# yassouali/pytorch-segmentation

Measured on NVIDIA H100. Metric: images/sec DeepLabV3+/ResNet101 513x513 train step (fwd+CE+bwd+SGD), higher is better.
Workload: dtype bf16

## Files before the change

### include/seg_b200.h

```cpp
#ifndef SEG_B200_H
#define SEG_B200_H

#include <stdint.h>

#ifdef __cplusplus
extern "C" {
#endif

#define SEG_DT_BF16 0
#define SEG_DT_F32 1

#define SEG_IMPL_AUTO 0
#define SEG_IMPL_SIMT 1
#define SEG_IMPL_TC 2

typedef struct seg_conv_desc {
  int32_t N, H, W, C;
  int32_t K;
  int32_t R, S;
  int32_t stride, pad, dil;
  int32_t P, Q;
  int32_t ldx;
  int32_t ldy;
} seg_conv_desc;

typedef struct seg_sync_desc {
  void* const* peers;
  int32_t rank, world, n_max;
  int64_t timeout_clocks;
} seg_sync_desc;

const char* seg_last_error(void);
int seg_version(void);
int seg_device_ok(void);
int64_t seg_launch_count(void);
void seg_launch_count_reset(void);

int seg_conv2d_fwd(const seg_conv_desc* d, const void* x, const void* w_packed, void* y, int y_dtype,
                   const float* bias, float beta, double* stats, const seg_sync_desc* sync, void* sync_ticket,
                   int impl, void* stream);
int seg_conv2d_dgrad(const seg_conv_desc* d, const void* dy, const void* w_packed, void* dx, float beta,
                     int impl, void* stream);
int64_t seg_conv2d_wgrad_workspace_floats(const seg_conv_desc* d, int impl);
int seg_conv2d_wgrad(const seg_conv_desc* d, const void* dy, const void* x, float* dw_packed, float* workspace, int impl,
                     void* stream);

int64_t seg_dwconv_scratch_floats(int C);
int seg_dwconv3x3_fwd(const seg_conv_desc* d, const void* x, const float* w9, void* y, double* stats,
                      const seg_sync_desc* sync, void* sync_ticket, void* stream);
int seg_dwconv3x3_bwd_data(const seg_conv_desc* d, const void* dy, const float* w9, void* dx, float beta, void* stream);
int seg_dwconv3x3_bwd_weight(const seg_conv_desc* d, const void* dy, const void* x, float* dw9, float beta,
                             float* scratch, void* stream);
int seg_dw_pack_weight(const float* w_c133, float* w9, int C, void* stream);
int seg_dw_unpack_wgrad(const float* g9, float* g_c133, int C, float beta, void* stream);

int seg_pack_weight(const float* w_oihw, void* w_packed, int K, int C, int R, int S, int Cpad, void* stream);
int seg_unpack_wgrad(const float* dw_packed, float* g_oihw, int K, int C, int R, int S, int Cpad, float beta,
                     void* stream);
int seg_pack_entry_bytes(void);
int seg_pack_weights_batched(const void* table, int n, int64_t total, void* stream);
int seg_unpack_wgrads_batched(const void* table, int n, int64_t total, float beta, void* stream);
int seg_im2col(const seg_conv_desc* d, const void* x, int x_nchw_f32, void* col, int Kpad, void* stream);

int seg_bn_stats(const void* x, int64_t M, int C, int ldx, double* stats, const seg_sync_desc* sync, void* sync_ticket,
                 void* stream);
int seg_bn_finalize(const double* stats, double count, int C, const float* gamma, const float* beta, float eps,
                    float momentum, int clamp_eps, float* running_mean, float* running_var, float* scale_shift,
                    float* save_mean_istd, void* stream);
// ... 177 lines not shown
```

### pytorch-segmentation_b200/csrc/seg_api.cu

```cuda
#include <stdarg.h>
#include "seg_common.cuh"
#include "seg_sync.cuh"

namespace seg {

static thread_local char g_err[1024] = "";
std::atomic<long long> g_launches{0};

void set_error(const char* fmt, ...) {
  va_list ap;
  va_start(ap, fmt);
  vsnprintf(g_err, sizeof(g_err), fmt, ap);
  va_end(ap);
}

namespace tc {
bool supported(const seg_conv_desc* d);
int conv_fwd(const seg_conv_desc* d, const void* x, const void* w, void* y, int y_dtype, const float* bias, float beta,
             double* stats, unsigned* stat_ticket, const seg_sync_desc* sync, cudaStream_t stream);
int conv_dgrad(const seg_conv_desc* d, const void* dy, const void* w, void* dx, float beta, cudaStream_t stream);
int conv_wgrad(const seg_conv_desc* d, const void* dy, const void* x, float* dw, float* ws, cudaStream_t stream);
int64_t wgrad_workspace_floats(const seg_conv_desc* d);
}
namespace simt {
int conv_fwd(const seg_conv_desc* d, const void* x, const void* w, void* y, int y_dtype, const float* bias, float beta,
             double* stats, unsigned* stat_ticket, const seg_sync_desc* sync, cudaStream_t stream);
int conv_dgrad(const seg_conv_desc* d, const void* dy, const void* w, void* dx, float beta, cudaStream_t stream);
int conv_wgrad(const seg_conv_desc* d, const void* dy, const void* x, float* dw, cudaStream_t stream);
}

static int check_desc(const seg_conv_desc* d) {
  SEG_REQUIRE(d != nullptr, "null conv descriptor");
  SEG_REQUIRE(d->N > 0 && d->H > 0 && d->W > 0 && d->C > 0 && d->K > 0 && d->R > 0 && d->S > 0, "bad conv dims");
  SEG_REQUIRE(d->stride >= 1 && d->dil >= 1 && d->pad >= 0, "bad conv stride/dil/pad");
  const int P = (d->H + 2 * d->pad - d->dil * (d->R - 1) - 1) / d->stride + 1;
  const int Q = (d->W + 2 * d->pad - d->dil * (d->S - 1) - 1) / d->stride + 1;
  SEG_REQUIRE(P == d->P && Q == d->Q, "conv output size mismatch: expected %dx%d got %dx%d", P, Q, d->P, d->Q);
  SEG_REQUIRE(d->ldx >= d->C && d->ldy >= d->K, "conv pitch smaller than channel count");
  return 0;
}

static bool tma_base_ok(const void* p) { return (reinterpret_cast<uintptr_t>(p) & 15) == 0; }

}

// ... 43 lines not shown
  const bool tc_ok = tc::supported(d) && d->ldy % 8 == 0 && tma_base_ok(dy) && tma_base_ok(w_packed);
  if (impl == SEG_IMPL_TC || (impl == SEG_IMPL_AUTO && tc_ok))
    return tc::conv_dgrad(d, dy, w_packed, dx, beta, ST(stream));
  return simt::conv_dgrad(d, dy, w_packed, dx, beta, ST(stream));
}

static bool wgrad_on_tc(const seg_conv_desc* d, int impl) {
  return impl == SEG_IMPL_TC || (impl == SEG_IMPL_AUTO && tc::supported(d) && d->ldy % 8 == 0);
}

int64_t seg_conv2d_wgrad_workspace_floats(const seg_conv_desc* d, int impl) {
  if (check_desc(d)) return -1;
  return wgrad_on_tc(d, impl) ? tc::wgrad_workspace_floats(d) : 0;
}

int seg_conv2d_wgrad(const seg_conv_desc* d, const void* dy, const void* x, float* dw_packed, float* workspace, int impl,
                     void* stream) {
  if (check_desc(d)) return 1;
  if (wgrad_on_tc(d, impl) && (impl == SEG_IMPL_TC || (tma_base_ok(dy) && tma_base_ok(x))))
    return tc::conv_wgrad(d, dy, x, dw_packed, workspace, ST(stream));
  return simt::conv_wgrad(d, dy, x, dw_packed, ST(stream));
}

}
```

### pytorch-segmentation_b200/csrc/seg_conv_tc.cu

```cuda
#include <cuda.h>
#include <mutex>
#include <stdlib.h>
#include "seg_common.cuh"
#include "seg_ptx.cuh"
#include "seg_sync.cuh"

namespace seg {
namespace tc {

using namespace ptx;

constexpr int BM = 128;
constexpr int BK = 64;
constexpr int A_BYTES = BM * 128;
constexpr int KIND_KK = 0, KIND_KM = 1;
constexpr int NTHREADS = 384;
constexpr int NCONS = 256;
constexpr int MAXT = 49;

constexpr int BAR_CONSUMERS = 1;
constexpr int BAR_ORDER = 2;
constexpr int BAR_WG = 4;

struct TcParams {
// ... 352 lines not shown
        }
        atomicAdd(p.stats + n0 + tid, (double)a);
        atomicAdd(p.stats + p.Ncols + n0 + tid, (double)b);
      }
    }
  }

  if (p.stats && p.sync.world > 0)
    sync_push_when_last<false>(p.sync, p.stats, 2 * p.Ncols, p.stat_ticket, gridDim.x, threadIdx.x - 128, NCONS,
                               [] { named_sync(BAR_CONSUMERS, NCONS); }, flag_sm);
}


template <int BN>
struct Cfg {
  static constexpr int B_BYTES = BN * 128;
  static constexpr int STAGE_BYTES = A_BYTES + B_BYTES;
  static constexpr int STAGES = BN == 64 ? 6 : (BN == 128 ? 5 : 4);
  static constexpr int SMEM = STAGES * STAGE_BYTES + 1024  + 256 ;
  static_assert(STAGES * STAGE_BYTES >= BM * BN * 4, "staging tile must fit in the pipeline ring");
  static_assert(SMEM <= 227 * 1024, "shared memory per block");
};

template <int BN>
__global__ void __launch_bounds__(NTHREADS, 1) conv_gemm_wgrad(const __grid_constant__ TcParams p) {
  using C = Cfg<BN>;
  constexpr int STAGES = C::STAGES;
  extern __shared__ uint8_t smem_raw[];
  const uint32_t raw_addr = smem_u32(smem_raw);
  const uint32_t smem0 = (raw_addr + 1023u) & ~1023u;
  uint8_t* smem_gen = smem_raw + (smem0 - raw_addr);
  const uint32_t bar0 = smem0 + STAGES * C::STAGE_BYTES;
  auto full_bar = [&](int s) { return bar0 + 8u * s; };
  auto empty_bar = [&](int s) { return bar0 + 8u * (STAGES + s); };

  const int m0 = blockIdx.x * BM;
  const int n0 = blockIdx.y * BN;

  const int tap_mm = blockIdx.z % p.taps;
  const int split = blockIdx.z / p.taps;
  const int kb_begin = split * p.kblocks_per_split;
  const int kb_end = min(kb_begin + p.kblocks_per_split, p.kblocks_total);
  const int num_iters = max(kb_end - kb_begin, 0);

  if (threadIdx.x == 0) {
    prefetch_tmap(&p.mapA);
    prefetch_tmap(&p.mapB);
    for (int s = 0; s < STAGES; ++s) {
      mbar_init(full_bar(s), 1);
      mbar_init(empty_bar(s), 8);
    }
    fence_mbar_init();
  }
  __syncthreads();
  pdl_wait();

  if (threadIdx.x < 128) {
    if (threadIdx.x == 0 && num_iters > 0) {
      const uint16_t oh = (uint16_t)p.tap_oh[tap_mm], ow = (uint16_t)p.tap_ow[tap_mm];
      int it = 0;
      for (int kb = kb_begin; kb < kb_end; ++kb, ++it) {
        const int st = it % STAGES;
        const uint32_t ph = (it / STAGES) & 1;
// ... 156 lines not shown
    SEG_REQUIRE(e == cudaSuccess, "cudaFuncSetAttribute(smem=%d): %s", PPCfg<BN>::SMEM, cudaGetErrorString(e));
    attr_set = true;
  }
  const int n_tiles = ceil_div(p.Ncols, BN);
  const int64_t tiles = ceil_div64(p.M, BM) * n_tiles;
  SEG_REQUIRE(tiles < (1ll << 31), "too many output tiles");
  p.n_tiles = n_tiles;
  p.tiles = (int)tiles;
  const dim3 grid((unsigned)std::min<int64_t>(tiles, num_sms()));
  launch_pdl(kfn, grid, dim3(NTHREADS), (size_t)PPCfg<BN>::SMEM, stream, p);
  return check_launch("conv_gemm_pp");
}

template <int KIND>
static int launch_pp_bn(int bn, TcParams& p, cudaStream_t stream) {
  switch (bn) {
    case 64: return launch_pp<64, KIND>(p, stream);
    case 128: return launch_pp<128, KIND>(p, stream);
  }
  set_error("bad BN %d", bn);
  return 1;
}

template <int BN>
static int launch_wgrad(const TcParams& p, dim3 grid, cudaStream_t stream) {
  static bool attr_set = false;
  auto kfn = conv_gemm_wgrad<BN>;
  if (!attr_set) {
    cudaError_t e = cudaFuncSetAttribute(kfn, cudaFuncAttributeMaxDynamicSharedMemorySize, Cfg<BN>::SMEM);
    SEG_REQUIRE(e == cudaSuccess, "cudaFuncSetAttribute(smem=%d): %s", Cfg<BN>::SMEM, cudaGetErrorString(e));
    attr_set = true;
  }
  launch_pdl(kfn, grid, dim3(NTHREADS), (size_t)Cfg<BN>::SMEM, stream, p);
  return check_launch("conv_gemm_wgrad");
}

static int launch_wgrad_bn(int bn, const TcParams& p, dim3 grid, cudaStream_t stream) {
  switch (bn) {
    case 64: return launch_wgrad<64>(p, grid, stream);
    case 128: return launch_wgrad<128>(p, grid, stream);
    case 256: return launch_wgrad<256>(p, grid, stream);
  }
  set_error("bad BN %d", bn);
  return 1;
}

static int pick_bn(int ncols, bool out_f32) { return (ncols <= 64 || out_f32) ? 64 : 128; }

static int stat_rows_for(int ncols) {
  if (ncols <= 64) return 32;
  if (ncols < 256) return 64;
  return ceil_div(ncols, 256) * 256 - ncols < 128 ? 128 : 64;
}

bool supported(const seg_conv_desc* d) {
  if (d->C % 8 != 0 || d->ldx % 8 != 0) return false;
  if (d->R != d->S) return false;
  if (d->R * d->S > MAXT) return false;
  if (d->pad > 127 || d->dil * (d->R - 1) - d->pad > 127 || d->dil * (d->R - 1) - d->pad < -127) return false;
  if (d->stride > 8) return false;
  return true;
}

static bool is_pointwise(const seg_conv_desc* d) { return d->R == 1 && d->S == 1 && d->stride == 1 && d->pad == 0; }
// ... 131 lines not shown
    dw[i] += acc;
  }
}

static void wgrad_plan(const seg_conv_desc* d, int& bn, int& splits, int& kblocks_per_split) {
  const bool wide = d->R * d->S >= 9 && d->C >= 256 && d->C % 256 == 0;
  bn = (d->C <= 64) ? 64 : (wide ? 256 : 128);
  const int kblocks_total = (int)ceil_div64((int64_t)d->N * d->P * d->Q, BK);
  const int tiles = ceil_div(d->K, BM) * ceil_div(d->C, bn) * d->R * d->S;
  splits = max(1, num_sms() / tiles);
  splits = min(splits, kblocks_total);
  splits = min(splits, 1024);
  kblocks_per_split = ceil_div(kblocks_total, splits);
  splits = ceil_div(kblocks_total, kblocks_per_split);
}

int64_t wgrad_workspace_floats(const seg_conv_desc* d) {
  if (!supported(d)) return 0;
  int bn, splits, kps;
  wgrad_plan(d, bn, splits, kps);
  return splits > 1 ? (int64_t)splits * d->R * d->S * d->K * d->C : 0;
}

int conv_wgrad(const seg_conv_desc* d, const void* dy, const void* x, float* dw, float* ws, cudaStream_t stream) {
  SEG_REQUIRE(supported(d) && d->ldy % 8 == 0, "wgmma conv wgrad: unsupported shape");
  TcParams p;
  memset(&p, 0, sizeof(p));
  const int64_t npix = (int64_t)d->N * d->P * d->Q;
  SEG_REQUIRE(npix < (1ll << 31), "too many pixels");
  p.M = d->K;
  p.Ncols = d->C;
  p.taps = d->R * d->S;
  for (int t = 0; t < p.taps; ++t) {
    p.tap_wt[t] = (short)t;
    p.tap_oh[t] = (short)((t / d->S) * d->dil);
    p.tap_ow[t] = (short)((t % d->S) * d->dil);
  }
  p.stride = d->stride;
  p.lower_h = p.lower_w = -d->pad;
  p.PQ = d->P * d->Q;
  p.Q = d->Q;
  p.dw = dw;
  p.dw_K = d->K;
  p.dw_C = d->C;
  p.kblocks_total = (int)ceil_div64(npix, BK);
  int bn, splits;
  wgrad_plan(d, bn, splits, p.kblocks_per_split);
  SEG_REQUIRE(splits == 1 || ws != nullptr, "wgmma conv wgrad: %d k-splits need the workspace (seg_conv2d_wgrad_workspace_floats)", splits);
  SEG_REQUIRE((int64_t)(splits - 1) * p.kblocks_per_split < p.kblocks_total, "wgmma conv wgrad: split %d has no k-blocks", splits - 1);
  if (splits > 1) p.ws = ws;
  if (make_map_2d(&p.mapA, dy, npix, d->K, d->ldy, 64)) return 1;
  if (is_pointwise(d)) {
    p.x_im2col = 0;
    if (make_map_2d(&p.mapB, x, npix, d->C, d->ldx, 64)) return 1;
  } else {
    p.x_im2col = 1;
    const int upper = d->pad - (d->R - 1) * d->dil;
    if (make_map_im2col(&p.mapB, x, d->N, d->H, d->W, d->C, d->ldx, -d->pad, -d->pad, upper, upper, d->stride, 64)) return 1;
  }
  SEG_REQUIRE((unsigned)(p.taps * splits) <= 65535u, "wgrad grid.z too large");
  dim3 grid((unsigned)ceil_div(d->K, BM), (unsigned)ceil_div(d->C, bn), (unsigned)(p.taps * splits));
  if (launch_wgrad_bn(bn, p, grid, stream)) return 1;
  if (splits == 1) return 0;
  const int64_t n = (int64_t)p.taps * d->K * d->C;
  wgrad_split_reduce_kernel<<<(unsigned)std::min<int64_t>(ceil_div64(n, 256), (int64_t)num_sms() * 8), 256, 0, stream>>>(ws, splits, n, dw);
  return check_launch("wgrad_split_reduce");
}

}
}
```

### pytorch-segmentation_b200/seg_b200/engine.py

```python
import torch

from . import ops
from .lib import IMPL_AUTO, IMPL_TC

BN_EPS = 1e-5
BN_MOM = 0.1
FUSED_BWD_MAX_BYTES = 24 << 20
ACT_DTYPE = torch.bfloat16


class Act:
    __slots__ = ("t", "grad", "needs_grad", "_written")

    def __init__(self, t, needs_grad=True):
        self.t = t
        self.grad = None
        self.needs_grad = needs_grad
        self._written = False

    @property
    def shape(self):
        return self.t.shape

    def grad_target(self):
# ... 54 lines not shown
        return self._packed


class DwSpec:

    def __init__(self, name, module):
        self.name, self.m = name, module
        assert module.groups == module.in_channels == module.out_channels and module.kernel_size == (3, 3)
        self.C = module.in_channels
        self._packed, self._version = None, None
        self.always_repack = False

    stride = property(lambda self: self.m.stride[0])
    pad = property(lambda self: self.m.padding[0])
    dil = property(lambda self: self.m.dilation[0])

    def packed(self):
        w = self.m.weight
        key = (w._version, w.data_ptr())
        if self._packed is None or self._version != key or self.always_repack:
            self._packed = ops.dw_pack_weight(w.detach())
            self._version = key
        return self._packed


class Tape:
    def __init__(self, training, record=None, grads=None, impl=IMPL_AUTO, dropout=True, seed=0, sync=None, clamp_eps=False,
                 step_ctr=None, arena_floats=0, owner=None):
        self.training = training
        self.record = training if record is None else record
        self.back = []
        self.back_params = {}
        self.grads = grads if grads is not None else {}
        self.touched = set()
        self.impl = impl
        self.dropout = dropout
        self.seed = seed
        self.sync = sync
        self.step_ctr = step_ctr
        self.packed_override = {}
        self.dw_buffers = {}
        self.clamp_eps = clamp_eps
        self._drop_ctr = 0
        self._pushed = set()
        self.bn_modules = []
        self.owner = owner
# ... 28 lines not shown
            return
        self.touched.add(p)
        if p in self.grads:
            value_fn(self.grads[p], 1.0)
        else:
            g = torch.empty(p.shape, dtype=torch.float32, device=p.device)
            value_fn(g, 0.0)
            self.grads[p] = g

    def _push_back(self, fn, params=()):
        if params:
            self.back_params[len(self.back)] = tuple(p for p in params if p is not None)
        self.back.append(fn)

    def backward(self, after=None):
        for i in range(len(self.back) - 1, -1, -1):
            self.back[i]()
            if after is not None:
                after(i)
        if self.owner is not None and self.arena_used:
            self.owner._arena_floats = self.arena_used
        self.back = []

    def conv(self, x, spec, out=None, out_dtype=None, want_stats=False, use_bias=True):
        wp = self.packed_override.get(spec)
        if wp is None:
            wp = spec.packed()
        bias = spec.m.bias if use_bias else None
        stats = None
        if out_dtype is None:
            out_dtype = ACT_DTYPE
        want = want_stats and self.training
        sync = tk = None
        if want:
            stats = self.zalloc64(2 * spec.K, wp.device)
            if self.sync_fused():
                sync, tk = self.sync, self.zalloc(1, wp.device)
        if spec.explicit:
            nchw = not isinstance(x, Act)
            if not nchw and self.record and x.needs_grad and (spec.R, spec.S, spec.stride, spec.pad) != (1, 1, 1, 0):
                raise NotImplementedError(f"{spec.name}: data gradient of an im2col conv is built for 1x1 convs only")
            src = x if nchw else x.t
            col = ops.im2col(src, spec.R, spec.S, spec.stride, spec.pad, spec.dil, spec.kpad, nchw_f32=nchw)
            y = ops.conv2d_fwd(col, wp, spec.K, 1, 1, out=out, out_dtype=out_dtype, bias=bias.detach() if bias is not None else None,
                               stats=stats, impl=self.impl, sync=sync, sync_ticket=tk)
            xin, geo = col, (1, 1, 1, 0, 1)
        else:
            y = ops.conv2d_fwd(x.t, wp, spec.K, spec.R, spec.S, spec.stride, spec.pad, spec.dil, out=out, out_dtype=out_dtype,
                               bias=bias.detach() if bias is not None else None, stats=stats, impl=self.impl, sync=sync, sync_ticket=tk)
            xin, geo = x.t, (spec.R, spec.S, spec.stride, spec.pad, spec.dil)
        ya = Act(y)
        if sync is not None:
            self._pushed.add(stats.data_ptr())
        if self.record:
            def bwd():
                dy = ya.grad
                if dy is None:
                    return
                R, S, stride, pad, dil = geo
                if spec.m.weight.requires_grad and spec in self.dw_buffers:
                    ops.conv2d_wgrad(dy, xin, R, S, stride, pad, dil, out=self.dw_buffers[spec], impl=self.impl)
                    self.touched.add(spec.m.weight)
                elif spec.m.weight.requires_grad:
                    dwp = ops.conv2d_wgrad(dy, xin, R, S, stride, pad, dil, impl=self.impl)
                    if spec.explicit:
                        def fill(g, beta):
                            full = dwp[0, :, : spec.R * spec.S * spec.C].reshape(spec.K, spec.R, spec.S, spec.C).permute(0, 3, 1, 2)
                            if beta:
                                g.add_(full)
                            else:
                                g.copy_(full)
                    else:
                        def fill(g, beta):
                            ops.unpack_wgrad(dwp, tuple(spec.m.weight.shape), beta=beta, out=g)
                    self._param_grad(spec.m.weight, fill)
                if bias is not None and bias.requires_grad:
                    cpad = ops.ld(dy)
                    wide = dy if dy.shape[-1] % 8 == 0 else dy.as_strided(dy.shape[:-1] + (cpad,), dy.stride(), dy.storage_offset())
                    s = ops.bn_stats(wide)[: spec.K].float()
                    self._param_grad(bias, lambda g, beta: g.add_(s) if beta else g.copy_(s))
                if (not spec.explicit) and isinstance(x, Act) and x.needs_grad:
                    gx, beta = x.grad_target()
                    ops.conv2d_dgrad(dy, wp, tuple(x.t.shape), R, S, stride, pad, dil, out=gx, beta=beta, impl=self.impl)
                elif isinstance(x, Act) and x.needs_grad:
                    assert x.grad is None, "the input of an im2col conv must have a single consumer"
                    x.grad = ops.conv2d_dgrad(dy, wp, tuple(xin.shape), 1, 1, 1, 0, 1, impl=self.impl)[..., : spec.C]
                    x._written = True
                ya.grad = None
            self._push_back(bwd, (spec.m.weight, bias))
        return ya, stats

    def conv_transpose(self, x, spec, out=None):
        assert spec.transposed
        wp = self.packed_override.get(spec)
        if wp is None:
            wp = spec.packed()
        impl = IMPL_TC if self.impl == IMPL_AUTO else self.impl
        k, s, p = spec.R, spec.stride, spec.pad
        N, h, w, _ = x.t.shape
        y_shape = (N, (h - 1) * s - 2 * p + k, (w - 1) * s - 2 * p + k, spec.C)
        y = ops.conv2d_dgrad(x.t, wp, y_shape, k, k, s, p, 1, out=out, impl=impl)
        ya = Act(y)
        if self.record:
            def bwd():
                dy = ya.grad
                if dy is None:
                    return
                if spec.m.weight.requires_grad and spec in self.dw_buffers:
                    ops.conv2d_wgrad(x.t, dy, k, k, s, p, 1, out=self.dw_buffers[spec], impl=impl)
                    self.touched.add(spec.m.weight)
                elif spec.m.weight.requires_grad:
                    dwp = ops.conv2d_wgrad(x.t, dy, k, k, s, p, 1, impl=impl)
# ... 422 lines not shown
```

### pytorch-segmentation_b200/seg_b200/lib.py

```python
import ctypes
import os
from ctypes import POINTER, Structure, c_char_p, c_double, c_float, c_int, c_int32, c_int64, c_uint8, c_uint32, c_uint64, c_void_p

import torch

_HERE = os.path.dirname(os.path.abspath(__file__))
LIB_PATH = os.path.join(os.path.dirname(_HERE), "libseg_b200.so")

DT_BF16, DT_F32 = 0, 1
IMPL_AUTO, IMPL_SIMT, IMPL_TC = 0, 1, 2
LOSS_CE, LOSS_WCE, LOSS_FOCAL = 0, 1, 2


class SyncDesc(Structure):

    _fields_ = [("peers", c_void_p), ("rank", c_int32), ("world", c_int32), ("n_max", c_int32), ("timeout_clocks", c_int64)]


class ConvDesc(Structure):

    _fields_ = [(n, c_int32) for n in ("N", "H", "W", "C", "K", "R", "S", "stride", "pad", "dil", "P", "Q", "ldx", "ldy")]


def conv_out_size(size, k, stride, pad, dil):
    return (size + 2 * pad - dil * (k - 1) - 1) // stride + 1


def make_conv_desc(N, H, W, C, K, R, S, stride, pad, dil, ldx=None, ldy=None):
    P = conv_out_size(H, R, stride, pad, dil)
    Q = conv_out_size(W, S, stride, pad, dil)
    return ConvDesc(N, H, W, C, K, R, S, stride, pad, dil, P, Q, ldx if ldx is not None else C, ldy if ldy is not None else K)


_SIGS = {
    "seg_last_error": (c_char_p, []),
    "seg_version": (c_int, []),
    "seg_device_ok": (c_int, []),
    "seg_launch_count": (c_int64, []),
    "seg_launch_count_reset": (None, []),
    "seg_conv2d_fwd": (c_int, [POINTER(ConvDesc), c_void_p, c_void_p, c_void_p, c_int, c_void_p, c_float, c_void_p, c_void_p, c_void_p, c_int, c_void_p]),
    "seg_conv2d_dgrad": (c_int, [POINTER(ConvDesc), c_void_p, c_void_p, c_void_p, c_float, c_int, c_void_p]),
    "seg_conv2d_wgrad_workspace_floats": (c_int64, [POINTER(ConvDesc), c_int]),
    "seg_conv2d_wgrad": (c_int, [POINTER(ConvDesc), c_void_p, c_void_p, c_void_p, c_void_p, c_int, c_void_p]),
    "seg_dwconv_scratch_floats": (c_int64, [c_int]),
    "seg_dwconv3x3_fwd": (c_int, [POINTER(ConvDesc), c_void_p, c_void_p, c_void_p, c_void_p, c_void_p, c_void_p, c_void_p]),
    "seg_dwconv3x3_bwd_data": (c_int, [POINTER(ConvDesc), c_void_p, c_void_p, c_void_p, c_float, c_void_p]),
    "seg_dwconv3x3_bwd_weight": (c_int, [POINTER(ConvDesc), c_void_p, c_void_p, c_void_p, c_float, c_void_p, c_void_p]),
    "seg_dw_pack_weight": (c_int, [c_void_p, c_void_p, c_int, c_void_p]),
    "seg_dw_unpack_wgrad": (c_int, [c_void_p, c_void_p, c_int, c_float, c_void_p]),
    "seg_pack_weight": (c_int, [c_void_p, c_void_p, c_int, c_int, c_int, c_int, c_int, c_void_p]),
    "seg_unpack_wgrad": (c_int, [c_void_p, c_void_p, c_int, c_int, c_int, c_int, c_int, c_float, c_void_p]),
    "seg_pack_entry_bytes": (c_int, []),
    "seg_pack_weights_batched": (c_int, [c_void_p, c_int, c_int64, c_void_p]),
    "seg_unpack_wgrads_batched": (c_int, [c_void_p, c_int, c_int64, c_float, c_void_p]),
    "seg_im2col": (c_int, [POINTER(ConvDesc), c_void_p, c_int, c_void_p, c_int, c_void_p]),
    "seg_bn_stats": (c_int, [c_void_p, c_int64, c_int, c_int, c_void_p, c_void_p, c_void_p, c_void_p]),
    "seg_bn_finalize": (c_int, [c_void_p, c_double, c_int, c_void_p, c_void_p, c_float, c_float, c_int, c_void_p, c_void_p, c_void_p, c_void_p, c_void_p]),
    "seg_bn_eval_scale_shift": (c_int, [c_int, c_void_p, c_void_p, c_void_p, c_void_p, c_float, c_void_p, c_void_p, c_void_p]),
    "seg_bn_apply": (c_int, [c_void_p, c_int, c_void_p, c_void_p, c_int, c_void_p, c_int, c_int64, c_int, c_int, c_float, c_uint64, c_void_p, c_int, c_void_p]),
    "seg_counter_add": (c_int, [c_void_p, c_uint64, c_void_p]),
    "seg_bn_bwd_reduce_slots": (c_int, []),
    "seg_bn_bwd_reduce": (c_int, [c_void_p, c_int, c_void_p, c_int, c_void_p, c_void_p, c_int, c_void_p, c_int64, c_int, c_int, c_float, c_void_p, c_void_p, c_void_p, c_void_p, c_void_p, c_int, c_void_p, c_void_p, c_void_p, c_void_p]),
    "seg_bn_apply_train": (c_int, [c_void_p, c_int, c_void_p, c_double, c_void_p, c_void_p, c_float, c_float, c_int, c_void_p, c_void_p, c_void_p, c_void_p, c_int, c_void_p, c_int, c_void_p, c_int64, c_int, c_int, c_float, c_uint64, c_void_p, c_int, c_void_p]),
    "seg_bn_bwd_fused_workspace": (c_int, [c_int64, c_int, POINTER(c_int64), POINTER(c_int64)]),
    "seg_bn_bwd_fused": (c_int, [c_void_p, c_int, c_void_p, c_int, c_void_p, c_void_p, c_int, c_void_p, c_void_p, c_void_p, c_double, c_int64, c_int, c_int, c_float,
                                 c_void_p, c_void_p, c_void_p, c_void_p, c_void_p, c_int, c_void_p, c_int, c_void_p, c_int, c_float, c_int, c_void_p, c_void_p]),
# ... 137 lines not shown
```

### pytorch-segmentation_b200/seg_b200/nets.py

```python
import logging
import math
import weakref
from itertools import chain

import numpy as np
import torch
import torch.nn as nn

from . import ops
from .engine import Act, BilinearHead, ConvSpec, DwSpec, FullResHead, ShuffleHead, Tape
from .lib import IMPL_AUTO, require_device

try:
    from base import BaseModel as _RefBaseModel
except Exception:
    _RefBaseModel = None


_LIVE_MODELS = weakref.WeakSet()


def release_all_graphs():
    import gc
    for m in list(_LIVE_MODELS):
        if hasattr(m, "release_graphs"):
            m.release_graphs()
    gc.collect()
    if torch.cuda.is_available():
        torch.cuda.synchronize()


class BaseModel(nn.Module if _RefBaseModel is None else _RefBaseModel):
    def __init__(self):
# ... 409 lines not shown
                               res=skip if last else None)
        return h

    def _new_tape(self, training, record):
        ctr = None
        if training:
            dev = next(self.parameters()).device
            if self._step_ctr is None or self._step_ctr.device != dev:
                bns = self._flat()[2]
                start = bns[0].num_batches_tracked.detach().reshape(1).to(dev, torch.int64) if bns else None
                self._step_ctr = start.clone() if start is not None else torch.zeros(1, dtype=torch.int64, device=dev)
            ctr = self._step_ctr
            ops.counter_add(ctr, 1)
        return Tape(training, record=record, impl=self.conv_impl, dropout=self.engine_dropout, seed=self._seed(),
                    sync=self.bn_sync, clamp_eps=self.syncbn_clamp_eps, step_ctr=ctr,
                    arena_floats=getattr(self, "_arena_floats", 0) if training else 0, owner=self)

    def _seed(self):
        if self.engine_seed is None:
            rank = torch.distributed.get_rank() if (torch.distributed.is_available() and torch.distributed.is_initialized()) else 0
            self.engine_seed = (int(torch.initial_seed()) * 2654435761 + rank * 0x9E3779B1) & 0x7FFFFFFF
        return self.engine_seed

    def _cbr(self, tape, x, name, conv, bn, relu=True, res=None, out=None, drop_p=0.0, drop_channelwise=False):
        y, st = tape.conv(x, self._spec(name, conv), want_stats=True)
        return tape.bn_act(y, bn, st, relu=relu, res=res, out=out, drop_p=drop_p, drop_channelwise=drop_channelwise)

    def _block(self, tape, x, prefix, blk, out=None):
        a = self._cbr(tape, x, prefix + "conv1", blk.conv1, blk.bn1)
        a = self._cbr(tape, a, prefix + "conv2", blk.conv2, blk.bn2)
        r = x
        if blk.downsample is not None:
            r = self._cbr(tape, x, prefix + "downsample.0", blk.downsample[0], blk.downsample[1], relu=False)
        return self._cbr(tape, a, prefix + "conv3", blk.conv3, blk.bn3, relu=True, res=r, out=out)

    def _finish(self, tape):
        if tape.bn_modules:
            torch._foreach_add_([m.num_batches_tracked for m in tape.bn_modules], 1)

    def _dp_world(self):
        if not self.dp_reduce:
            return 1
        from .comm import dp_world
        return dp_world()

    def _attach_sync_bn(self):
        from . import comm
        if self.use_sync_bn and self.bn_sync is None and comm.dp_world() > 1:
# ... 106 lines not shown
            a = self._xblock(tape, a, f"backbone.block{i}.", getattr(bb, f"block{i}"), relu_out=True)
        for n in (3, 4, 5):
            a = self._sep_unit(tape, a, f"backbone.conv{n}", getattr(bb, f"conv{n}"), getattr(bb, f"bn{n}"), relu_after=True)
        return a, low

    def _trunk_resnet(self, tape, x):
        bb = self.backbone
        a = self._cbr(tape, x, "backbone.layer0.0", bb.layer0[0], bb.layer0[1])
        a = tape.maxpool(a)
        low = None
        for li in (1, 2, 3, 4):
            layer = getattr(bb, f"layer{li}")
            for bi, blk in enumerate(layer):
                a = self._block(tape, a, f"backbone.layer{li}.{bi}.", blk)
            if li == 1:
                low = a
        return a, low

    def _aspp(self, tape, a):
        N, Hf, Wf = a.t.shape[0], a.t.shape[1], a.t.shape[2]
        A = self.ASSP
        cat, sl = tape.concat(N, Hf, Wf, [256] * 5, a.t.device)
        br = []
        for i in (1, 2, 3, 4):
            seq = getattr(A, f"aspp{i}")
            br.append(self._cbr(tape, a, f"ASSP.aspp{i}.0", seq[0], seq[1], out=sl[i - 1]))
        g = tape.avgpool(a, 1)
        g = self._cbr(tape, g, "ASSP.avg_pool.1", A.avg_pool[1], A.avg_pool[2])
        br.append(tape.bilinear(g, Hf, Wf, True, out=sl[4]))
        tape.bind_slices(cat, br)
        return self._cbr(tape, cat, "ASSP.conv1", A.conv1, A.bn1, drop_p=A.dropout.p)

    def _decoder(self, tape, f, low):
        D = self.decoder
        N, Hl, Wl = low.t.shape[0], low.t.shape[1], low.t.shape[2]
        cat2, sl2 = tape.concat(N, Hl, Wl, [48, 256], low.t.device)
        l48 = self._cbr(tape, low, "decoder.conv1", D.conv1, D.bn1, out=sl2[0])
        up = tape.bilinear(f, Hl, Wl, True, out=sl2[1])
        tape.bind_slices(cat2, [l48, up])
        y = self._cbr(tape, cat2, "decoder.output.0", D.output[0], D.output[1])
        y = self._cbr(tape, y, "decoder.output.3", D.output[3], D.output[4], drop_p=D.output[6].p)
        lo, _ = tape.conv(y, self._spec("decoder.output.7", D.output[7]), out_dtype=torch.float32)
        return lo

    def _features(self, tape, x):
        a, low = self._trunk_xception(tape, x) if self.backbone_name == "xception" else self._trunk_resnet(tape, x)
        return self._decoder(tape, self._aspp(tape, a), low)

    def _forward_heads(self, tape, x):
# ... 242 lines not shown
            for p in self.backbone.parameters():
                p.requires_grad = False

    def _decoder(self, tape, f, low):
        D = self.decoder
        N, Hl, Wl = low.t.shape[0], low.t.shape[1], low.t.shape[2]
        cat, sl = tape.concat(N, Hl, Wl, [48, 256], low.t.device)
        l48 = self._cbr(tape, low, "decoder.conv1", D.conv1, D.bn1, out=sl[0])
        u = self._cbr(tape, f, "decoder.DUC.conv", D.DUC.conv, D.DUC.bn)
        up = tape.pixel_shuffle(u, 2, out=sl[1], crop=(Hl, Wl))
        tape.bind_slices(cat, [l48, up])
        y = self._cbr(tape, cat, "decoder.output.0", D.output[0], D.output[1])
        y = self._cbr(tape, y, "decoder.output.3", D.output[3], D.output[4], drop_p=D.output[6].p)
        C = self.num_classes
        buf = torch.empty((N, Hl, Wl, (C + 7) // 8 * 8), dtype=y.t.dtype, device=y.t.device)[..., :C]
        lo, _ = tape.conv(y, self._spec("decoder.output.7", D.output[7]), out=buf)
        return lo

    def _aspp(self, tape, a):
        N, Hf, Wf = a.t.shape[0], a.t.shape[1], a.t.shape[2]
        A = self.ASSP
        cat, sl = tape.concat(N, Hf, Wf, [256] * 7, a.t.device)
        br = []
        for i in range(1, 7):
            seq = getattr(A, f"aspp{i}")
            br.append(self._cbr(tape, a, f"ASSP.aspp{i}.0", seq[0], seq[1], out=sl[i - 1]))
        g = tape.avgpool(a, 1)
        g = self._cbr(tape, g, "ASSP.avg_pool.1", A.avg_pool[1], A.avg_pool[2])
        br.append(tape.bilinear(g, Hf, Wf, True, out=sl[6]))
        tape.bind_slices(cat, br)
        return self._cbr(tape, cat, "ASSP.conv1", A.conv1, A.bn1, drop_p=A.dropout.p)

    def _forward_heads(self, tape, x):
        bb = self.backbone
        a = self._cbr(tape, x, "backbone.layer0.0", bb.layer0[0], bb.layer0[1])
        a = tape.maxpool(a)
        low = None
        for li in (1, 2, 3, 4):
            for bi, blk in enumerate(getattr(bb, f"layer{li}")):
                a = self._block(tape, a, f"backbone.layer{li}.{bi}.", blk)
            if li == 1:
                low = a
        y = self._decoder(tape, self._aspp(tape, a), low)
        z = self._cbr(tape, y, "DUC_out.conv", self.DUC_out.conv, self.DUC_out.bn)
        return [ShuffleHead(z, 4)]

    def get_backbone_params(self):
        return self.backbone.parameters()

# ... 297 lines not shown
```

### pytorch-segmentation_b200/seg_b200/ops.py

```python
import ctypes

import torch

from . import lib
from .lib import DT_BF16, DT_F32, IMPL_AUTO, IMPL_SIMT, IMPL_TC, ConvDesc, call, make_conv_desc, ptr

_IMPL_OVERRIDE = None
PROFILE = None


def _meta(d):
    if lib.TRACE is None:
        return None
    return (d.N, d.H, d.W, d.C, d.K, d.R, d.stride, d.dil, 2.0 * d.N * d.P * d.Q * d.K * d.C * d.R * d.S)


def _meta_rows(M, C, passes, flag=0):
    if lib.TRACE is None:
        return None
    return (int(M), int(C), int(flag), 0, 0, 0, 0, 0, 2.0 * M * C * passes)


def _prof(kind, d):
    if PROFILE is None:
        return None
    e0, e1 = torch.cuda.Event(enable_timing=True), torch.cuda.Event(enable_timing=True)
    flops = 2.0 * d.N * d.P * d.Q * d.K * d.C * d.R * d.S
    nbytes = 2.0 * (d.N * d.H * d.W * d.C + d.N * d.P * d.Q * d.K) + (4.0 if kind == "wgrad" else 2.0) * d.K * d.C * d.R * d.S
    PROFILE.append((kind, flops, e0, e1, nbytes))
    e0.record()
    return e1


def set_conv_impl(impl):
    global _IMPL_OVERRIDE
    _IMPL_OVERRIDE = impl


def _impl(impl):
    return _IMPL_OVERRIDE if _IMPL_OVERRIDE is not None else impl


def ld(t):
    assert t.stride(-1) == 1, "channel dim must be contiguous"
    if t.dim() == 4:
        n, h, w, c = t.shape
        pitch = t.stride(2) if w > 1 else (t.stride(1) // w if h > 1 else (t.stride(0) // (h * w) if n > 1 else c))
        assert w == 1 or t.stride(2) == pitch
        assert h == 1 or t.stride(1) == w * pitch, "rows must be dense"
        assert n == 1 or t.stride(0) == h * w * pitch, "images must be dense"
        return pitch
# ... 73 lines not shown
    ev = _prof("dgrad", d)
    call("seg_conv2d_dgrad", ctypes.byref(d), ptr(dy), ptr(w_packed), ptr(out), float(beta), _impl(impl), meta=_meta(d))
    if ev is not None:
        ev.record()
    return out


def conv2d_wgrad(dy, x, R, S, stride=1, pad=0, dil=1, out=None, impl=IMPL_AUTO):
    N, H, W, C = x.shape
    K = dy.shape[-1]
    if out is None:
        out = torch.zeros((R * S, K, C), dtype=torch.float32, device=x.device)
    d = make_conv_desc(N, H, W, C, K, R, S, stride, pad, dil, ldx=ld(x), ldy=ld(dy))
    assert (d.P, d.Q) == (dy.shape[1], dy.shape[2])
    nws = lib.load().seg_conv2d_wgrad_workspace_floats(ctypes.byref(d), _impl(impl))
    if nws < 0:
        raise RuntimeError(f"seg_conv2d_wgrad_workspace_floats failed: {lib.last_error()}")
    ws = torch.empty(nws, dtype=torch.float32, device=x.device) if nws > 0 else None
    ev = _prof("wgrad", d)
    call("seg_conv2d_wgrad", ctypes.byref(d), ptr(dy), ptr(x), ptr(out), ptr(ws), _impl(impl), meta=_meta(d))
    if ev is not None:
        ev.record()
    return out


def dw_pack_weight(w_c133):
    C = w_c133.shape[0]
    w9 = torch.empty((9, C), dtype=torch.float32, device=w_c133.device)
    call("seg_dw_pack_weight", ptr(w_c133), ptr(w9), C)
    return w9


def dw_unpack_wgrad(g9, out, beta=0.0):
    call("seg_dw_unpack_wgrad", ptr(g9), ptr(out), g9.shape[1], float(beta))
    return out


def _dw_desc(x_shape, stride, pad, dil, ldx, ldy):
    N, H, W, C = x_shape
    return make_conv_desc(N, H, W, C, C, 3, 3, stride, pad, dil, ldx=ldx, ldy=ldy)


def dwconv_fwd(x, w9, stride=1, pad=1, dil=1, out=None, stats=None, sync=None, sync_ticket=None):
    N, H, W, C = x.shape
    d = _dw_desc(x.shape, stride, pad, dil, ld(x), C)
    if out is None:
# ... 652 lines not shown
```

Measured before the change: 383.1.

## Batch ASPP dilated-branch weight gradients into one grouped wgrad launch

Adds a grouped weight-gradient GEMM kernel that packs up to six same-shape conv problems, each with its own dy, pad, dilation and output, into one grid, with blockIdx.z mapped to the member problem. The ASPP 3x3 dilated branches share the same input, so their wgrads are deferred until the last branch's backward runs and are then issued as a single launch. The goal is to fill the GPU better on small per-branch wgrad grids and to cut launch overhead. The cost is a larger grid-constant parameter block, a linear search over groups in each block, and more complex backward bookkeeping for deferral and parameter ownership.

Result: no change. 385.5, median of 6 (+0.6%).

```diff
diff --git a/include/seg_b200.h b/include/seg_b200.h
--- a/include/seg_b200.h
+++ b/include/seg_b200.h
@@ -44,6 +44,10 @@
 int64_t seg_conv2d_wgrad_workspace_floats(const seg_conv_desc* d, int impl);
 int seg_conv2d_wgrad(const seg_conv_desc* d, const void* dy, const void* x, float* dw_packed, float* workspace, int impl,
                      void* stream);
+#define SEG_WGRAD_GROUP_MAX 6
+int64_t seg_conv2d_wgrad_group_workspace_floats(const seg_conv_desc* d, int G, int impl);
+int seg_conv2d_wgrad_group(const seg_conv_desc* d, int G, const void* const* dy, const void* x, float* const* dw_packed,
+                           float* workspace, int impl, void* stream);
 
 int64_t seg_dwconv_scratch_floats(int C);
 int seg_dwconv3x3_fwd(const seg_conv_desc* d, const void* x, const float* w9, void* y, double* stats,
diff --git a/pytorch-segmentation_b200/csrc/seg_api.cu b/pytorch-segmentation_b200/csrc/seg_api.cu
--- a/pytorch-segmentation_b200/csrc/seg_api.cu
+++ b/pytorch-segmentation_b200/csrc/seg_api.cu
@@ -21,6 +21,10 @@
 int conv_dgrad(const seg_conv_desc* d, const void* dy, const void* w, void* dx, float beta, cudaStream_t stream);
 int conv_wgrad(const seg_conv_desc* d, const void* dy, const void* x, float* dw, float* ws, cudaStream_t stream);
 int64_t wgrad_workspace_floats(const seg_conv_desc* d);
+bool wgrad_group_compatible(const seg_conv_desc* d, int G);
+int64_t wgrad_group_workspace_floats(const seg_conv_desc* d, int G);
+int conv_wgrad_group(const seg_conv_desc* d, int G, const void* const* dy, const void* x, float* const* dw, float* ws,
+                     cudaStream_t stream);
 }
 namespace simt {
 int conv_fwd(const seg_conv_desc* d, const void* x, const void* w, void* y, int y_dtype, const float* bias, float beta,
@@ -110,4 +114,39 @@
   return simt::conv_wgrad(d, dy, x, dw_packed, ST(stream));
 }
 
+static bool wgrad_group_on_tc(const seg_conv_desc* d, int G, int impl) {
+  return (impl == SEG_IMPL_TC || impl == SEG_IMPL_AUTO) && tc::wgrad_group_compatible(d, G);
 }
+
+int64_t seg_conv2d_wgrad_group_workspace_floats(const seg_conv_desc* d, int G, int impl) {
+  if (G < 1 || G > SEG_WGRAD_GROUP_MAX) {
+    seg::set_error("wgrad group: G = %d outside 1..%d", G, SEG_WGRAD_GROUP_MAX);
+    return -1;
+  }
+  int64_t n = 0;
+  for (int i = 0; i < G; ++i) {
+    const int64_t ni = seg_conv2d_wgrad_workspace_floats(&d[i], impl);
+    if (ni < 0) return -1;
+    n += ni;
+  }
+  return n;
+}
+
+int seg_conv2d_wgrad_group(const seg_conv_desc* d, int G, const void* const* dy, const void* x, float* const* dw_packed,
+                           float* workspace, int impl, void* stream) {
+  if (G < 1 || G > SEG_WGRAD_GROUP_MAX) {
+    seg::set_error("wgrad group: G = %d outside 1..%d", G, SEG_WGRAD_GROUP_MAX);
+    return 1;
+  }
+  for (int i = 0; i < G; ++i)
+    if (check_desc(&d[i])) return 1;
+  bool aligned = tma_base_ok(x);
+  for (int i = 0; i < G; ++i) aligned = aligned && tma_base_ok(dy[i]);
+  if (wgrad_group_on_tc(d, G, impl) && (impl == SEG_IMPL_TC || aligned))
+    return tc::conv_wgrad_group(d, G, dy, x, dw_packed, workspace, ST(stream));
+  for (int i = 0; i < G; ++i)
+    if (seg_conv2d_wgrad(&d[i], dy[i], x, dw_packed[i], workspace, impl, stream)) return 1;
+  return 0;
+}
+
+}
diff --git a/pytorch-segmentation_b200/csrc/seg_conv_tc.cu b/pytorch-segmentation_b200/csrc/seg_conv_tc.cu
--- a/pytorch-segmentation_b200/csrc/seg_conv_tc.cu
+++ b/pytorch-segmentation_b200/csrc/seg_conv_tc.cu
@@ -398,8 +398,21 @@
   static_assert(SMEM <= 227 * 1024, "shared memory per block");
 };
 
-template <int BN>
-__global__ void __launch_bounds__(NTHREADS, 1) conv_gemm_wgrad(const __grid_constant__ TcParams p) {
+constexpr int MAXG = SEG_WGRAD_GROUP_MAX;
+template <int G>
+struct WgradGroup {
+  TcParams p[G];
+  int z_end[G];
+  int count;
+};
+
+template <int BN, int G>
+__global__ void __launch_bounds__(NTHREADS, 1) conv_gemm_wgrad(const __grid_constant__ WgradGroup<G> g) {
+  int gi = 0;
+  if constexpr (G > 1)
+    while (gi + 1 < g.count && (int)blockIdx.z >= g.z_end[gi]) ++gi;
+  const TcParams& p = g.p[gi];
+  const int bz = (int)blockIdx.z - (gi > 0 ? g.z_end[gi - 1] : 0);
   using C = Cfg<BN>;
   constexpr int STAGES = C::STAGES;
   extern __shared__ uint8_t smem_raw[];
@@ -413,8 +426,8 @@
   const int m0 = blockIdx.x * BM;
   const int n0 = blockIdx.y * BN;
 
-  const int tap_mm = blockIdx.z % p.taps;
-  const int split = blockIdx.z / p.taps;
+  const int tap_mm = bz % p.taps;
+  const int split = bz / p.taps;
   const int kb_begin = split * p.kblocks_per_split;
   const int kb_end = min(kb_begin + p.kblocks_per_split, p.kblocks_total);
   const int num_iters = max(kb_end - kb_begin, 0);
@@ -617,24 +630,25 @@
   return 1;
 }
 
-template <int BN>
-static int launch_wgrad(const TcParams& p, dim3 grid, cudaStream_t stream) {
+template <int BN, int G>
+static int launch_wgrad(const WgradGroup<G>& g, dim3 grid, cudaStream_t stream) {
   static bool attr_set = false;
-  auto kfn = conv_gemm_wgrad<BN>;
+  auto kfn = conv_gemm_wgrad<BN, G>;
   if (!attr_set) {
     cudaError_t e = cudaFuncSetAttribute(kfn, cudaFuncAttributeMaxDynamicSharedMemorySize, Cfg<BN>::SMEM);
     SEG_REQUIRE(e == cudaSuccess, "cudaFuncSetAttribute(smem=%d): %s", Cfg<BN>::SMEM, cudaGetErrorString(e));
     attr_set = true;
   }
-  launch_pdl(kfn, grid, dim3(NTHREADS), (size_t)Cfg<BN>::SMEM, stream, p);
+  launch_pdl(kfn, grid, dim3(NTHREADS), (size_t)Cfg<BN>::SMEM, stream, g);
   return check_launch("conv_gemm_wgrad");
 }
 
-static int launch_wgrad_bn(int bn, const TcParams& p, dim3 grid, cudaStream_t stream) {
+template <int G>
+static int launch_wgrad_bn(int bn, const WgradGroup<G>& g, dim3 grid, cudaStream_t stream) {
   switch (bn) {
-    case 64: return launch_wgrad<64>(p, grid, stream);
-    case 128: return launch_wgrad<128>(p, grid, stream);
-    case 256: return launch_wgrad<256>(p, grid, stream);
+    case 64: return launch_wgrad<64, G>(g, grid, stream);
+    case 128: return launch_wgrad<128, G>(g, grid, stream);
+    case 256: return launch_wgrad<256, G>(g, grid, stream);
   }
   set_error("bad BN %d", bn);
   return 1;
@@ -812,9 +826,9 @@
   return splits > 1 ? (int64_t)splits * d->R * d->S * d->K * d->C : 0;
 }
 
-int conv_wgrad(const seg_conv_desc* d, const void* dy, const void* x, float* dw, float* ws, cudaStream_t stream) {
+static int wgrad_params(const seg_conv_desc* d, const void* dy, const void* x, float* dw, float* ws, TcParams& p, int& bn,
+                        int& splits) {
   SEG_REQUIRE(supported(d) && d->ldy % 8 == 0, "wgmma conv wgrad: unsupported shape");
-  TcParams p;
   memset(&p, 0, sizeof(p));
   const int64_t npix = (int64_t)d->N * d->P * d->Q;
   SEG_REQUIRE(npix < (1ll << 31), "too many pixels");
@@ -834,7 +848,6 @@
   p.dw_K = d->K;
   p.dw_C = d->C;
   p.kblocks_total = (int)ceil_div64(npix, BK);
-  int bn, splits;
   wgrad_plan(d, bn, splits, p.kblocks_per_split);
   SEG_REQUIRE(splits == 1 || ws != nullptr, "wgmma conv wgrad: %d k-splits need the workspace (seg_conv2d_wgrad_workspace_floats)", splits);
   SEG_REQUIRE((int64_t)(splits - 1) * p.kblocks_per_split < p.kblocks_total, "wgmma conv wgrad: split %d has no k-blocks", splits - 1);
@@ -848,14 +861,73 @@
     const int upper = d->pad - (d->R - 1) * d->dil;
     if (make_map_im2col(&p.mapB, x, d->N, d->H, d->W, d->C, d->ldx, -d->pad, -d->pad, upper, upper, d->stride, 64)) return 1;
   }
-  SEG_REQUIRE((unsigned)(p.taps * splits) <= 65535u, "wgrad grid.z too large");
-  dim3 grid((unsigned)ceil_div(d->K, BM), (unsigned)ceil_div(d->C, bn), (unsigned)(p.taps * splits));
-  if (launch_wgrad_bn(bn, p, grid, stream)) return 1;
+  return 0;
+}
+
+static int wgrad_reduce(const seg_conv_desc* d, int splits, const float* ws, float* dw, cudaStream_t stream) {
   if (splits == 1) return 0;
-  const int64_t n = (int64_t)p.taps * d->K * d->C;
+  const int64_t n = (int64_t)d->R * d->S * d->K * d->C;
   wgrad_split_reduce_kernel<<<(unsigned)std::min<int64_t>(ceil_div64(n, 256), (int64_t)num_sms() * 8), 256, 0, stream>>>(ws, splits, n, dw);
   return check_launch("wgrad_split_reduce");
 }
 
-}
-}
+int conv_wgrad(const seg_conv_desc* d, const void* dy, const void* x, float* dw, float* ws, cudaStream_t stream) {
+  WgradGroup<1> g;
+  int bn, splits;
+  if (wgrad_params(d, dy, x, dw, ws, g.p[0], bn, splits)) return 1;
+  SEG_REQUIRE((unsigned)(g.p[0].taps * splits) <= 65535u, "wgrad grid.z too large");
+  g.z_end[0] = g.p[0].taps * splits;
+  g.count = 1;
+  dim3 grid((unsigned)ceil_div(d->K, BM), (unsigned)ceil_div(d->C, bn), (unsigned)g.z_end[0]);
+  if (launch_wgrad_bn(bn, g, grid, stream)) return 1;
+  return wgrad_reduce(d, splits, ws, dw, stream);
+}
+
+bool wgrad_group_compatible(const seg_conv_desc* d, int G) {
+  if (G < 1 || G > MAXG) return false;
+  for (int i = 0; i < G; ++i) {
+    const seg_conv_desc& a = d[0];
+    const seg_conv_desc& b = d[i];
+    if (!supported(&b) || b.ldy % 8 != 0) return false;
+    if (b.N != a.N || b.H != a.H || b.W != a.W || b.C != a.C || b.K != a.K || b.R != a.R || b.S != a.S ||
+        b.stride != a.stride || b.P != a.P || b.Q != a.Q || b.ldx != a.ldx)
+      return false;
+  }
+  return true;
+}
+
+int64_t wgrad_group_workspace_floats(const seg_conv_desc* d, int G) {
+  int64_t n = 0;
+  for (int i = 0; i < G; ++i) n += wgrad_workspace_floats(&d[i]);
+  return n;
+}
+
+int conv_wgrad_group(const seg_conv_desc* d, int G, const void* const* dy, const void* x, float* const* dw, float* ws,
+                     cudaStream_t stream) {
+  SEG_REQUIRE(wgrad_group_compatible(d, G), "wgmma conv wgrad group: %d problems that do not share one grid", G);
+  WgradGroup<MAXG> g;
+  memset(&g, 0, sizeof(g));
+  g.count = G;
+  int bn = 0, splits[MAXG];
+  float* wsi = ws;
+  int z = 0;
+  for (int i = 0; i < G; ++i) {
+    int bni;
+    if (wgrad_params(&d[i], dy[i], x, dw[i], wsi, g.p[i], bni, splits[i])) return 1;
+    SEG_REQUIRE(i == 0 || bni == bn, "wgmma conv wgrad group: tile widths differ");
+    bn = bni;
+    if (splits[i] > 1) wsi += wgrad_workspace_floats(&d[i]);
+    z += g.p[i].taps * splits[i];
+    g.z_end[i] = z;
+  }
+  SEG_REQUIRE((unsigned)z <= 65535u, "wgrad grid.z too large");
+  dim3 grid((unsigned)ceil_div(d[0].K, BM), (unsigned)ceil_div(d[0].C, bn), (unsigned)z);
+  if (launch_wgrad_bn(bn, g, grid, stream)) return 1;
+  for (int i = 0; i < G; ++i) {
+    if (wgrad_reduce(&d[i], splits[i], g.p[i].ws, dw[i], stream)) return 1;
+  }
+  return 0;
+}
+
+}
+}
diff --git a/pytorch-segmentation_b200/seg_b200/engine.py b/pytorch-segmentation_b200/seg_b200/engine.py
--- a/pytorch-segmentation_b200/seg_b200/engine.py
+++ b/pytorch-segmentation_b200/seg_b200/engine.py
@@ -100,6 +100,37 @@
             self._packed = ops.dw_pack_weight(w.detach())
             self._version = key
         return self._packed
+
+
+class WgradGroup:
+
+    def __init__(self):
+        self.members = []
+        self.pending = []
+        self.back_index = None
+
+    def flush(self, tape):
+        todo, self.pending = self.pending, []
+        if not todo:
+            return
+        _, _, x, (R, S, stride, _, _) = todo[0]
+        outs = []
+        for spec, dy, _, _ in todo:
+            if spec in tape.dw_buffers:
+                outs.append(tape.dw_buffers[spec])
+                tape.touched.add(spec.m.weight)
+            else:
+                outs.append(torch.zeros((R * S, dy.shape[-1], x.shape[-1]), dtype=torch.float32, device=x.device))
+        group = getattr(ops, "conv2d_wgrad_group", None)
+        if group is not None:
+            group([t[1] for t in todo], x, R, S, stride, [t[3][3] for t in todo], [t[3][4] for t in todo], outs, impl=tape.impl)
+        else:
+            for (_, dy, _, (_, _, _, pad, dil)), o in zip(todo, outs):
+                ops.conv2d_wgrad(dy, x, R, S, stride, pad, dil, out=o, impl=tape.impl)
+        for (spec, _, _, _), dwp in zip(todo, outs):
+            if spec not in tape.dw_buffers:
+                tape._param_grad(spec.m.weight, lambda g, beta, dwp=dwp, spec=spec: ops.unpack_wgrad(
+                    dwp, tuple(spec.m.weight.shape), beta=beta, out=g))
 
 
 class Tape:
@@ -174,7 +205,7 @@
             self.owner._arena_floats = self.arena_used
         self.back = []
 
-    def conv(self, x, spec, out=None, out_dtype=None, want_stats=False, use_bias=True):
+    def conv(self, x, spec, out=None, out_dtype=None, want_stats=False, use_bias=True, wgrad_group=None):
         wp = self.packed_override.get(spec)
         if wp is None:
             wp = spec.packed()
@@ -204,13 +235,23 @@
         ya = Act(y)
         if sync is not None:
             self._pushed.add(stats.data_ptr())
+        grp = wgrad_group if (wgrad_group is not None and not spec.explicit and spec.m.weight.requires_grad) else None
+        if grp is not None:
+            grp.members.append(spec)
         if self.record:
             def bwd():
                 dy = ya.grad
+                last = grp is not None and grp.members[0] is spec
                 if dy is None:
+                    if last:
+                        grp.flush(self)
                     return
                 R, S, stride, pad, dil = geo
-                if spec.m.weight.requires_grad and spec in self.dw_buffers:
+                if grp is not None:
+                    grp.pending.append((spec, dy, xin, geo))
+                    if last:
+                        grp.flush(self)
+                elif spec.m.weight.requires_grad and spec in self.dw_buffers:
                     ops.conv2d_wgrad(dy, xin, R, S, stride, pad, dil, out=self.dw_buffers[spec], impl=self.impl)
                     self.touched.add(spec.m.weight)
                 elif spec.m.weight.requires_grad:
@@ -239,7 +280,14 @@
                     x.grad = ops.conv2d_dgrad(dy, wp, tuple(xin.shape), 1, 1, 1, 0, 1, impl=self.impl)[..., : spec.C]
                     x._written = True
                 ya.grad = None
-            self._push_back(bwd, (spec.m.weight, bias))
+            if grp is None:
+                self._push_back(bwd, (spec.m.weight, bias))
+            elif grp.members[0] is spec:
+                grp.back_index = len(self.back)
+                self._push_back(bwd, (spec.m.weight, bias))
+            else:
+                self._push_back(bwd, (bias,) if bias is not None else ())
+                self.back_params[grp.back_index] += (spec.m.weight,)
         return ya, stats
 
     def conv_transpose(self, x, spec, out=None):
diff --git a/pytorch-segmentation_b200/seg_b200/lib.py b/pytorch-segmentation_b200/seg_b200/lib.py
--- a/pytorch-segmentation_b200/seg_b200/lib.py
+++ b/pytorch-segmentation_b200/seg_b200/lib.py
@@ -42,6 +42,8 @@
     "seg_conv2d_dgrad": (c_int, [POINTER(ConvDesc), c_void_p, c_void_p, c_void_p, c_float, c_int, c_void_p]),
     "seg_conv2d_wgrad_workspace_floats": (c_int64, [POINTER(ConvDesc), c_int]),
     "seg_conv2d_wgrad": (c_int, [POINTER(ConvDesc), c_void_p, c_void_p, c_void_p, c_void_p, c_int, c_void_p]),
+    "seg_conv2d_wgrad_group_workspace_floats": (c_int64, [POINTER(ConvDesc), c_int, c_int]),
+    "seg_conv2d_wgrad_group": (c_int, [POINTER(ConvDesc), c_int, POINTER(c_void_p), c_void_p, POINTER(c_void_p), c_void_p, c_int, c_void_p]),
     "seg_dwconv_scratch_floats": (c_int64, [c_int]),
     "seg_dwconv3x3_fwd": (c_int, [POINTER(ConvDesc), c_void_p, c_void_p, c_void_p, c_void_p, c_void_p, c_void_p, c_void_p]),
     "seg_dwconv3x3_bwd_data": (c_int, [POINTER(ConvDesc), c_void_p, c_void_p, c_void_p, c_float, c_void_p]),
diff --git a/pytorch-segmentation_b200/seg_b200/nets.py b/pytorch-segmentation_b200/seg_b200/nets.py
--- a/pytorch-segmentation_b200/seg_b200/nets.py
+++ b/pytorch-segmentation_b200/seg_b200/nets.py
@@ -8,7 +8,7 @@
 import torch.nn as nn
 
 from . import ops
-from .engine import Act, BilinearHead, ConvSpec, DwSpec, FullResHead, ShuffleHead, Tape
+from .engine import Act, BilinearHead, ConvSpec, DwSpec, FullResHead, ShuffleHead, Tape, WgradGroup
 from .lib import IMPL_AUTO, require_device
 
 try:
@@ -464,8 +464,8 @@
             self.engine_seed = (int(torch.initial_seed()) * 2654435761 + rank * 0x9E3779B1) & 0x7FFFFFFF
         return self.engine_seed
 
-    def _cbr(self, tape, x, name, conv, bn, relu=True, res=None, out=None, drop_p=0.0, drop_channelwise=False):
-        y, st = tape.conv(x, self._spec(name, conv), want_stats=True)
+    def _cbr(self, tape, x, name, conv, bn, relu=True, res=None, out=None, drop_p=0.0, drop_channelwise=False, wgrad_group=None):
+        y, st = tape.conv(x, self._spec(name, conv), want_stats=True, wgrad_group=wgrad_group)
         return tape.bn_act(y, bn, st, relu=relu, res=res, out=out, drop_p=drop_p, drop_channelwise=drop_channelwise)
 
     def _block(self, tape, x, prefix, blk, out=None):
@@ -618,9 +618,11 @@
         A = self.ASSP
         cat, sl = tape.concat(N, Hf, Wf, [256] * 5, a.t.device)
         br = []
+        grp = WgradGroup()
         for i in (1, 2, 3, 4):
             seq = getattr(A, f"aspp{i}")
-            br.append(self._cbr(tape, a, f"ASSP.aspp{i}.0", seq[0], seq[1], out=sl[i - 1]))
+            br.append(self._cbr(tape, a, f"ASSP.aspp{i}.0", seq[0], seq[1], out=sl[i - 1],
+                                wgrad_group=grp if seq[0].kernel_size == (3, 3) else None))
         g = tape.avgpool(a, 1)
         g = self._cbr(tape, g, "ASSP.avg_pool.1", A.avg_pool[1], A.avg_pool[2])
         br.append(tape.bilinear(g, Hf, Wf, True, out=sl[4]))
@@ -909,9 +911,11 @@
         A = self.ASSP
         cat, sl = tape.concat(N, Hf, Wf, [256] * 7, a.t.device)
         br = []
+        grp = WgradGroup()
         for i in range(1, 7):
             seq = getattr(A, f"aspp{i}")
-            br.append(self._cbr(tape, a, f"ASSP.aspp{i}.0", seq[0], seq[1], out=sl[i - 1]))
+            br.append(self._cbr(tape, a, f"ASSP.aspp{i}.0", seq[0], seq[1], out=sl[i - 1],
+                                wgrad_group=grp if seq[0].kernel_size == (3, 3) else None))
         g = tape.avgpool(a, 1)
         g = self._cbr(tape, g, "ASSP.avg_pool.1", A.avg_pool[1], A.avg_pool[2])
         br.append(tape.bilinear(g, Hf, Wf, True, out=sl[6]))
diff --git a/pytorch-segmentation_b200/seg_b200/ops.py b/pytorch-segmentation_b200/seg_b200/ops.py
--- a/pytorch-segmentation_b200/seg_b200/ops.py
+++ b/pytorch-segmentation_b200/seg_b200/ops.py
@@ -21,12 +21,12 @@
     return (int(M), int(C), int(flag), 0, 0, 0, 0, 0, 2.0 * M * C * passes)
 
 
-def _prof(kind, d):
+def _prof(kind, d, count=1):
     if PROFILE is None:
         return None
     e0, e1 = torch.cuda.Event(enable_timing=True), torch.cuda.Event(enable_timing=True)
-    flops = 2.0 * d.N * d.P * d.Q * d.K * d.C * d.R * d.S
-    nbytes = 2.0 * (d.N * d.H * d.W * d.C + d.N * d.P * d.Q * d.K) + (4.0 if kind == "wgrad" else 2.0) * d.K * d.C * d.R * d.S
+    flops = 2.0 * d.N * d.P * d.Q * d.K * d.C * d.R * d.S * count
+    nbytes = 2.0 * (d.N * d.H * d.W * d.C + count * d.N * d.P * d.Q * d.K) + count * (4.0 if kind == "wgrad" else 2.0) * d.K * d.C * d.R * d.S
     PROFILE.append((kind, flops, e0, e1, nbytes))
     e0.record()
     return e1
@@ -146,6 +146,26 @@
     if ev is not None:
         ev.record()
     return out
+
+
+def conv2d_wgrad_group(dys, x, R, S, stride, pads, dils, outs, impl=IMPL_AUTO):
+    G = len(dys)
+    N, H, W, C = x.shape
+    descs = (ConvDesc * G)(*[make_conv_desc(N, H, W, C, dy.shape[-1], R, S, stride, pads[i], dils[i], ldx=ld(x), ldy=ld(dy))
+                             for i, dy in enumerate(dys)])
+    for d, dy in zip(descs, dys):
+        assert (d.P, d.Q) == (dy.shape[1], dy.shape[2])
+    nws = lib.load().seg_conv2d_wgrad_group_workspace_floats(descs, G, _impl(impl))
+    if nws < 0:
+        raise RuntimeError(f"seg_conv2d_wgrad_group_workspace_floats failed: {lib.last_error()}")
+    ws = torch.empty(nws, dtype=torch.float32, device=x.device) if nws > 0 else None
+    dy_ptrs = (ctypes.c_void_p * G)(*[ptr(dy) for dy in dys])
+    dw_ptrs = (ctypes.c_void_p * G)(*[ptr(o) for o in outs])
+    ev = _prof("wgrad", descs[0], G)
+    call("seg_conv2d_wgrad_group", descs, G, dy_ptrs, ptr(x), dw_ptrs, ptr(ws), _impl(impl), meta=_meta(descs[0]))
+    if ev is not None:
+        ev.record()
+    return outs
 
 
 def dw_pack_weight(w_c133):
```
